# ODD2/DFD-CLIP

Hardware: AMD Instinct MI355X
Metric: 1-sec clips/sec (30x224x224 frames) ViT-B/16 (higher is better)
Workload: dtype bf16

## Files before the change

### dfd-clip_amd/capi.py

```python
import ctypes
import os
from ctypes import POINTER, Structure, c_char_p, c_float, c_int, c_int32, c_int64, c_size_t, c_uint32, c_void_p

import torch

PKG_DIR = os.path.dirname(os.path.abspath(__file__))
LIB_PATH = os.path.join(PKG_DIR, "libdfdclip_hip.so")

F32, BF16 = 0, 1
EPI_BIAS, EPI_BIAS_QUICKGELU, EPI_BIAS_RESIDUAL, EPI_PATCH_EMBED, EPI_QKV_EXPORT, EPI_RESIDUAL_POS, EPI_BIAS_GELU = range(7)
ABI_VERSION = 17

_DTYPE = {torch.float32: F32, torch.bfloat16: BF16}
FP8 = 2
FP8_MAX = 448.0
FP8_MIN_ROWS = 1024


class DfdError(RuntimeError):
    pass


GEMM_STREAM_OUT = 1
GEMM_SPARE_IF_FREE = 2


class GemmExtra(Structure):
    _fields_ = [("pos", c_void_p), ("cls", c_void_p), ("k_export", c_void_p), ("v_export", c_void_p),
                ("tokens", c_int32), ("frames_per_clip", c_int32), ("residual", c_void_p), ("qkv_first", c_int32),
                ("drop_rng", c_void_p), ("drop_site", c_uint32), ("drop_p", c_float), ("flags", c_uint32)]


class DropoutDesc(Structure):
    _fields_ = [("rng_state", c_void_p), ("site", c_uint32), ("p", c_float)]


class Dropout:
    __slots__ = ("rng", "site", "p")

# ... 196 lines not shown
    _profile["events"] = []
    _profile["base"] = None
    if epilogue is not None:
        _profile["base"] = torch.cuda.Event(enable_timing=True)
        _profile["base"].record()


def profile_gemm_collect():
    base = _profile["base"]
    spans = [(base.elapsed_time(a), base.elapsed_time(b), flops) for a, b, flops in _profile["events"]]
    profile_gemm(None)
    return spans


def gemm(a, w, c, bias=None, epilogue=EPI_BIAS, m=None, pos=None, cls=None, k_export=None, v_export=None, tokens=0,
         frames_per_clip=0, residual=None, qkv_first=0, drop=None, stream_out=False, spare_cus=0, tile_blocks=0, spare_if_free=False):
    _dev(a, w, c, bias, pos, cls, k_export, v_export, residual)
    assert a.dtype == w.dtype and a.stride(1) == 1 and w.stride(1) == 1 and c.stride(1) == 1
    M = a.shape[0] if m is None else m
    N, K = w.shape
    assert a.shape[1] == K
    assert residual is None or (residual.dtype == c.dtype and residual.stride(0) == c.stride(0))
    assert drop is None or epilogue == EPI_RESIDUAL_POS
    assert 0 <= epilogue <= EPI_BIAS_GELU, f"unknown epilogue {epilogue}"
    extra = GemmExtra(_ptr(pos).value, _ptr(cls).value, _ptr(k_export).value, _ptr(v_export).value, tokens, frames_per_clip,
                      _ptr(residual).value, qkv_first, drop.rng.data_ptr() if drop is not None and drop.p > 0 else None,
                      drop.site if drop is not None else 0, drop.p if drop is not None else 0.0, (GEMM_STREAM_OUT if stream_out else 0) | (GEMM_SPARE_IF_FREE if spare_if_free else 0) | ((int(spare_cus) & 0xff) << 8) | ((int(tile_blocks) & 0xf) << 16))
    timed = _profile["epilogue"] == epilogue
    if timed:
        e0, e1 = torch.cuda.Event(enable_timing=True), torch.cuda.Event(enable_timing=True)
        e0.record()
    _check(load_library().dfd_gemm(_ptr(a), a.stride(0), _ptr(w), w.stride(0), _DTYPE[a.dtype], _ptr(c), c.stride(0),
                                   _DTYPE[c.dtype], _ptr(bias), epilogue, ctypes.byref(extra), M, N, K, _stream()), "dfd_gemm")
    if timed:
        e1.record()
        _profile["events"].append((e0, e1, 2.0 * M * N * K))
    return c


def gemm_fp8(a, w, c, col_scale, bias=None, epilogue=EPI_BIAS, m=None, out_inv_scale=0.0, pos=None, k_export=None, v_export=None,
             tokens=0, frames_per_clip=0, qkv_first=0, stream_out=False, spare_cus=0, spare_if_free=False):
    _dev(a, w, c, col_scale, bias, pos, k_export, v_export)
# ... 363 lines not shown
```

### dfd-clip_amd/csrc/gemm.hip

```cpp
#include "gemm_args.hpp"
#include "gelu.hpp"

namespace {

constexpr int BM = 128, BN = 128;
constexpr int ROW_BYTES = 64;
constexpr int ROW_STRIDE = 80;
constexpr int TILE_BYTES = BM * ROW_STRIDE;
constexpr int EPI_SPLITK_SLAB = 100;

template <typename CT> __device__ __forceinline__ void store_c(void* C, int64_t off, float v) {
  static_cast<CT*>(C)[off] = from_f32<CT>(v);
}

template <typename CT, int EPI>
__device__ __forceinline__ void epilogue_elem(const GemmArgs& a, int64_t m, int n, float acc) {
  if (m >= a.M || n >= a.N) return;
  if constexpr (EPI == DFD_EPI_BIAS) {
    store_c<CT>(a.C, m * a.ldc + n, acc + (a.bias ? a.bias[n] : 0.f));
  } else if constexpr (EPI == DFD_EPI_BIAS_QUICKGELU) {
    store_c<CT>(a.C, m * a.ldc + n, quick_gelu(acc + (a.bias ? a.bias[n] : 0.f)));
  } else if constexpr (EPI == DFD_EPI_BIAS_GELU) {
    store_c<CT>(a.C, m * a.ldc + n, gelu_erf(acc + (a.bias ? a.bias[n] : 0.f)));
  } else if constexpr (EPI == DFD_EPI_BIAS_RESIDUAL) {
// ... 250 lines not shown
    DFD_REQUIRE(!extra->k_export == !extra->v_export, "dfd_gemm: QKV_EXPORT needs both k_export and v_export or neither");
    DFD_REQUIRE(!extra->pos || extra->frames_per_clip > 0, "dfd_gemm: QKV_EXPORT with pos needs frames_per_clip");
  }
  if (epilogue == DFD_EPI_RESIDUAL_POS) {
    DFD_REQUIRE(extra && extra->tokens > 1, "dfd_gemm: RESIDUAL_POS needs extra.tokens (patches per frame + 1)");
    DFD_REQUIRE(!extra->pos || extra->frames_per_clip > 0, "dfd_gemm: RESIDUAL_POS with pos needs frames_per_clip");
  }
  if (extra) {
    a.pos = extra->pos; a.cls = extra->cls; a.k_export = extra->k_export; a.v_export = extra->v_export;
    a.residual = epilogue == DFD_EPI_RESIDUAL_POS ? extra->residual : nullptr;
    a.tokens = extra->tokens; a.frames_per_clip = extra->frames_per_clip > 0 ? extra->frames_per_clip : 1;
    a.qkv_first = epilogue == DFD_EPI_QKV_EXPORT ? extra->qkv_first : 0;
    a.stream_out = (extra->flags & DFD_GEMM_STREAM_OUT) ? 1 : 0;
    a.spare_cus = (int)((extra->flags >> DFD_GEMM_SPARE_CUS_SHIFT) & 0xff);
    a.spare_if_free = (extra->flags & DFD_GEMM_SPARE_IF_FREE) ? 1 : 0;
    a.tile_rows = 32 * (int)((extra->flags >> DFD_GEMM_TILE_BLOCKS_SHIFT) & 0xf);
    DFD_REQUIRE(a.tile_rows == 0 || a.tile_rows == 224 || a.tile_rows == 256, "dfd_gemm: tile blocks must be 0, 7 or 8");
    if (epilogue == DFD_EPI_RESIDUAL_POS && extra->drop_rng && extra->drop_p > 0.f) {
      DFD_REQUIRE(extra->drop_p < 1.f, "dfd_gemm: drop_p=%f", (double)extra->drop_p);
      const dfd_dropout_t dd{extra->drop_rng, extra->drop_site, extra->drop_p};
      a.drop = dfd_make_drop(&dd);
    }
  }
  return DFD_OK;
}

static thread_local int g_last_path = 0;
static thread_local int g_gemm_variant = 0;
extern "C" int dfd_gemm_last_path(void) { return g_last_path; }
extern "C" int dfd_gemm_set_variant(int variant) {
// ... 11 lines not shown
  DFD_REQUIRE(c_dtype == DFD_F32 || c_dtype == DFD_BF16, "dfd_gemm: c_dtype=%d", c_dtype);
  DFD_REQUIRE(!(ab_dtype == DFD_F32 && c_dtype == DFD_BF16), "dfd_gemm: f32 operands with bf16 output unsupported");
  DFD_REQUIRE(K % 32 == 0, "dfd_gemm: K=%d must be a multiple of 32", K);
  const int esz = ab_dtype == DFD_F32 ? 4 : 2;
  DFD_REQUIRE(lda >= K && ldw >= K && (lda * esz) % 16 == 0 && (ldw * esz) % 16 == 0, "dfd_gemm: lda=%lld ldw=%lld must be >= K and 16-byte multiples", (long long)lda, (long long)ldw);
  DFD_REQUIRE(dfd_aligned16(A) && dfd_aligned16(W), "dfd_gemm: A and W must be 16-byte aligned");
  GemmArgs a{};
  a.A = A; a.W = W; a.C = C; a.bias = bias;
  a.lda = lda; a.ldw = ldw; a.ldc = ldc; a.M = M; a.N = N; a.K = K;
  { const int rc = fill_extra(a, epilogue, extra, c_dtype, ldc, M, N); if (rc != DFD_OK) return rc; }
  if (M == 0) return DFD_OK;
  hipStream_t st = static_cast<hipStream_t>(stream);
  if (ab_dtype == DFD_BF16) {
    const int epi_p = epilogue == DFD_EPI_QKV_EXPORT && a.k_export == nullptr ? DFD_EPI_BIAS : epilogue;
    a.no_dynamic = g_gemm_variant != 3;
    int rc = g_gemm_variant == 1 ? 1 : dfd_gemm256e_try(a, c_dtype, epi_p, st);
    if (rc == 0) g_last_path = 257;
    if (rc <= 0) return rc;
    rc = dfd_gemm256p_try(a, c_dtype, epi_p, st);
    if (rc == 0) g_last_path = 256;
    if (rc <= 0) return rc;
    rc = dfd_gemm256_try(a, c_dtype, epilogue, st);
    if (rc == 0) g_last_path = 256;
    if (rc <= 0) return rc;
  }
  g_last_path = 128;
  if (ab_dtype == DFD_F32) return launch_gemm128<float, float>(a, epilogue, st);
  if (c_dtype == DFD_BF16) return launch_gemm128<bf16_t, bf16_t>(a, epilogue, st);
  return launch_gemm128<bf16_t, float>(a, epilogue, st);
}

extern "C" int dfd_gemm_fp8(const void* A, int64_t lda, const void* W, int64_t ldw, void* C, int64_t ldc, int c_dtype,
                            const float* col_scale, const float* bias, float out_inv_scale, int epilogue,
                            const dfd_gemm_extra* extra, int64_t M, int N, int K, void* stream) {
// ... 59 lines not shown
```

### dfd-clip_amd/csrc/gemm256e.hip

```cpp
#include <mutex>
#include <unordered_map>

#include "gemm256p_common.hpp"
#include "gelu.hpp"

namespace {

constexpr int UNIT = 128 * ROWB;
constexpr int DEPTH = 6;
constexpr int NB = 2 * (DEPTH - 1);

template <int EPI, int RB, bool F8, bool CF8>
__global__ __launch_bounds__(512) void gemm256e_kernel(const GemmArgs a, int tiles_m, int tiles_n) {
  static_assert(!F8 || RB == 8, "fp8 form: 256-row tiles only");
  static_assert(!CF8 || (F8 && EPI != DFD_EPI_QKV_EXPORT), "fp8 output: fp8 operands, plain or QuickGELU epilogue");
  constexpr int ESZ = F8 ? 1 : 2;
  constexpr int CSZ = CF8 ? 1 : 2;
  constexpr int TMU = 32 * RB;
  constexpr int WROWS = 16 * RB;
  constexpr int HB = RB - 4;
  constexpr int NCV = F8 ? 2 : 1;
  constexpr int S1 = CF8 ? RB : 2 * RB;
  constexpr int S2 = 4 * RB;
  __shared__ __attribute__((aligned(1024))) unsigned char smem[RING + 8 * STAGE];
  const int tid = threadIdx.x;
  const int lane = tid & 63;
  const int wave = __builtin_amdgcn_readfirstlane(tid >> 6);
  const int wr = wave >> 2, wc = wave & 3;
  const int ntiles = tiles_m * tiles_n;

  const int G = gridDim.x, bid = blockIdx.x;
  const int xcd = bid & 7, q8 = G >> 3, r8 = G & 7;
  const int pos = (xcd < r8 ? xcd * (q8 + 1) : r8 * (q8 + 1) + (xcd - r8) * q8) + (bid >> 3);

  const __amdgpu_buffer_rsrc_t srdA = __builtin_amdgcn_make_buffer_rsrc(const_cast<void*>(a.A), 0, (int)(uint32_t)(a.M * a.lda * ESZ), 0x00020000);
  const __amdgpu_buffer_rsrc_t srdW = __builtin_amdgcn_make_buffer_rsrc(const_cast<void*>(a.W), 0, (int)(uint32_t)((int64_t)a.N * a.ldw * ESZ), 0x00020000);
  const __amdgpu_buffer_rsrc_t srdC = __builtin_amdgcn_make_buffer_rsrc(a.C, 0, (int)(uint32_t)(a.M * a.ldc * CSZ), 0x00020000);
  auto words = [](const float* p, int bytes) {
    const uint64_t u = reinterpret_cast<uint64_t>(p);
    return v4i{(int)(uint32_t)u, (int)((uint32_t)(u >> 32) & 0xffffu), bytes, 0x00020000};
  };
  const v4i srdB = words(a.bias ? a.bias : reinterpret_cast<const float*>(a.W), a.bias ? a.N * 4 : 0);
  [[maybe_unused]] const v4i srdS = words(F8 ? a.col_scale : reinterpret_cast<const float*>(a.W), F8 ? a.N * 4 : 0);
  const int cnt_x = q8 + (xcd < r8 ? 1 : 0), off_x = pos - (bid >> 3);
  const v4i srdT = words(reinterpret_cast<const float*>(a.sched ? a.sched : reinterpret_cast<const uint32_t*>(a.W)), a.sched ? 8 * 128 : 0);

  const uint32_t lda2 = (uint32_t)(a.lda * ESZ), ldw2 = (uint32_t)(a.ldw * ESZ);
  const uint32_t a_last = (uint32_t)(a.M - 1) * lda2;
  uint32_t vA[2][2], vW[2];
  auto set_a = [&](const Tile& t, int ha) {
    int l = lane;
    asm volatile("" : "+v"(l));
// ... 75 lines not shown
      for (int ks = 0; ks < 2; ++ks)
#pragma unroll
        for (int i = 0; i < (ha == 0 ? 4 : HB); ++i)
#pragma unroll
          for (int j = 0; j < 2; ++j)
            acc[4 * ha + i][2 * hb + j] = __builtin_amdgcn_mfma_f32_16x16x32_bf16(chunk(w[j], ks), chunk(Aa[i], ks), acc[4 * ha + i][2 * hb + j], 0, 0, 0);
    }
    __builtin_amdgcn_s_setprio(0);
    __builtin_amdgcn_sched_barrier(0);
    __builtin_amdgcn_s_barrier();
    __builtin_amdgcn_sched_barrier(0);
  };

  const int nk = a.K / (F8 ? 128 : TK);
  int idx = pos;
  Tile cur = decode_tile(idx, tiles_m, tiles_n, TMU);
  set_a(cur, 0);
  set_a(cur, 1);
  set_w(cur, 0);
  set_w(cur, 1);
#pragma unroll
  for (int v = 0; v <= DEPTH; ++v) issue(v & 3, v >> 2);
  wait_vm<NB>();
  __builtin_amdgcn_s_barrier();
  if (wr == 1) __builtin_amdgcn_s_barrier();
  __builtin_amdgcn_sched_barrier(0);
  int s_prev = 0;

  [[maybe_unused]] unsigned char* const ep = smem + RING + wave * STAGE;
  const int D = EPI == DFD_EPI_QKV_EXPORT ? a.N / (3 - a.qkv_first) : 0;
  [[maybe_unused]] __amdgpu_buffer_rsrc_t srdK = srdC, srdV = srdC, srdP = srdC;
// ... 1 lines not shown
    if (a.k_export != nullptr) {
      srdP = __builtin_amdgcn_make_buffer_rsrc(const_cast<float*>(a.pos ? a.pos : reinterpret_cast<const float*>(a.W)), 0,
                                               a.pos ? a.frames_per_clip * D * 4 : 0, 0x00020000);
      const int64_t erows = (a.M / a.tokens) * (a.tokens - 1);
      srdK = __builtin_amdgcn_make_buffer_rsrc(a.k_export, 0, (int)(uint32_t)(erows * D * 2), 0x00020000);
      srdV = __builtin_amdgcn_make_buffer_rsrc(a.v_export, 0, (int)(uint32_t)(erows * D * 2), 0x00020000);
    }
  }

  const int nk_ = a.K / (F8 ? 128 : TK);
  const bool dyn = !F8 && a.sched != nullptr && nk_ >= 6;
  const bool drawer = dyn && wave == 0;
  for (;;) {
    int nidx = idx + G;
    bool has_next = nidx < ntiles;
    Tile nxt = has_next ? decode_tile(nidx, tiles_m, tiles_n, TMU) : cur;
    uint32_t drawn = 1;
    if (drawer) {
      const uint32_t coff = (uint32_t)(xcd * 128);
      uint64_t saved_exec;
      asm volatile(
          "s_mov_b64 %1, exec\n\t"
          "s_mov_b64 exec, 1\n\t"
          "s_nop 4\n\t"
          "buffer_atomic_add %0, %2, %3, 0 offen sc0\n\t"
          "s_mov_b64 exec, %1"
          : "+v"(drawn), "=&s"(saved_exec)
          : "v"(coff), "s"(srdT)
          : "memory");
    }
#pragma unroll
// ... 99 lines not shown
        ktile(2, C0{}, C2{}, C1{});
        ktile(3, C1{}, C2{}, C0{});
      }
    } else {
      ktile(0, C0{}, C0{}, C4{});
      ktile(1, C1{}, C1{}, C4{});
      if (dyn) {
        uint32_t n;
        const uint32_t slot_addr = (uint32_t)(uintptr_t)(lds_ptr_t)(smem + RING + 1024);
        asm volatile("ds_read_b32 %0, %1\n\ts_waitcnt lgkmcnt(0)" : "=&v"(n) : "v"(slot_addr) : "memory");
        n = (uint32_t)__builtin_amdgcn_readfirstlane((int)n) - a.sched_base[xcd];
        const uint32_t r = n / (uint32_t)cnt_x;
        has_next = r < (uint32_t)(ntiles / G + 1);
        nidx = (int)((r + 1) * (uint32_t)G + (uint32_t)off_x + (n - r * (uint32_t)cnt_x));
        has_next = has_next && nidx < ntiles;
        nxt = has_next ? decode_tile(nidx, tiles_m, tiles_n, TMU) : cur;
      }
      for (int kt = 2; kt < nk - 4; kt += 2) {
        ktile(kt, C0{}, C2{}, C4{});
        ktile(kt + 1, C1{}, C2{}, C4{});
      }
      ktile(nk - 4, C0{}, C2{}, C3{});
      ktile(nk - 3, C1{}, C2{}, C2{});
      ktile(nk - 2, C0{}, C2{}, C1{});
      ktile(nk - 1, C1{}, C2{}, C0{});
    }

    int le = lane;
    asm volatile("" : "+v"(le));
    const int er = le & 15, eq = le >> 4;
    const int drow = le >> 3, dc = le & 7;
// ... 6 lines not shown
    int stores = 2 * RB;
    {
      f32x4 b4[4];
      [[maybe_unused]] f32x4 cs4[4];
#pragma unroll
      for (int j = 0; j < 4; ++j) {
        b4[j] = *reinterpret_cast<const f32x4*>(ep + (j * 16 + eq * 4) * 4);
        if constexpr (F8) cs4[j] = *reinterpret_cast<const f32x4*>(ep + 256 + (j * 16 + eq * 4) * 4);
      }
      asm volatile("s_waitcnt lgkmcnt(0)" ::: "memory");
#pragma unroll
      for (int i = 0; i < RB; ++i)
#pragma unroll
        for (int j = 0; j < 4; ++j) {
          if constexpr (F8) acc[i][j] = acc[i][j] * cs4[j] + b4[j];
          else acc[i][j] += b4[j];
        }
      if constexpr (EPI == DFD_EPI_QKV_EXPORT) {
        if (exporting) {
          stores = 4 * RB;
          const int ecol = nb - (which - a.qkv_first) * D + dc * 8;
          unsigned char* const parkf = ep + er * 256;
          const __amdgpu_buffer_rsrc_t srdE = which == 2 ? srdV : srdK;
#pragma unroll
          for (int i = 0; i < RB; ++i) {
            __builtin_amdgcn_sched_barrier(0);
            uint32_t eoff[2];
            f32x4 pe[2][2];
#pragma unroll
            for (int rr = 0; rr < 2; ++rr) {
              const int rloc = i * 16 + rr * 8;
// ... 97 lines not shown
            for (int e = 0; e < 4; ++e) {
              dv[e] = x0[e];
              dv[4 + e] = x1[e];
            }
            dfd_drop_eight(a.drop, (uint64_t)gq[b][rr] << 3, dv);
            const bf16x8 ob = __builtin_bit_cast(bf16x8, oq[b][rr]);
            bf16x8 o;
#pragma unroll
            for (int e = 0; e < 4; ++e) {
              o[e] = (bf16_t)((float)ob[e] + dv[e] + pq[b][rr][0][e]);
              o[4 + e] = (bf16_t)((float)ob[4 + e] + dv[4 + e] + pq[b][rr][1][e]);
            }
            store_out(__builtin_bit_cast(v4i, o), srdC, offq[b][rr], a.stream_out);
          }
        }
      } else if constexpr (CF8) {
        stores = RB;
        const int srow = le >> 2, sc = le & 3;
        unsigned char* const park8 = ep + er * 64 + eq * 4;
        const int psw = (er >> 1) & 3;
        const unsigned char* const dsrc8 = ep + srow * 64 + ((sc ^ ((srow >> 1) & 3)) << 4);
        const int64_t m8 = (int64_t)cur.m0 + wr * WROWS + srow;
        const int rows_left8 = (int)min((int64_t)0x7fffffff, a.M - m8);
        const uint32_t cbase8 = (uint32_t)(m8 * a.ldc + nb + sc * 16);
#pragma unroll
        for (int q = 0; q < 4; ++q) {
#pragma unroll
          for (int ii = 0; ii < 2; ++ii) {
            const int i = 2 * q + ii;
#pragma unroll
// ... 110 lines not shown
  if (n_cu == 0) {
    int dev = 0;
    hipDeviceProp_t prop;
    if (hipGetDevice(&dev) != hipSuccess || hipGetDeviceProperties(&prop, dev) != hipSuccess) {
      dfd_set_error("dfd_gemm(ping-pong): cannot query the device");
      return DFD_ERR_LAUNCH;
    }
    n_cu = prop.multiProcessorCount;
  }
  int cus = n_cu - a.spare_cus;
  cus = cus < n_cu / 2 ? n_cu / 2 : cus;
  if (a.spare_cus > 0 && a.spare_if_free) {
    auto cost = [&](int c) {
      auto r = [&](int rows) { return (double)((((a.M + rows - 1) / rows) * tiles_n + c - 1) / c); };
      const double r256 = r(256), r224 = r(224) * 0.97;
      return (F8 || EPI == DFD_EPI_RESIDUAL_POS) ? (EPI == DFD_EPI_RESIDUAL_POS ? r224 : r256) : (r224 < r256 ? r224 : r256);
    };
    if (cost(cus) > cost(n_cu)) cus = n_cu;
  }
  auto rounds = [&](int rows) {
    const int64_t tiles = ((a.M + rows - 1) / rows) * tiles_n;
    return (double)((tiles + cus - 1) / cus);
  };
  const bool use224 = !F8 && (EPI == DFD_EPI_RESIDUAL_POS || a.tile_rows == 224 || (a.tile_rows == 0 && rounds(224) * 0.97 < rounds(256)));
  const int rows = use224 ? 224 : 256;
  const int tiles_m = (int)((a.M + rows - 1) / rows);
  const int64_t ntiles = (int64_t)tiles_m * tiles_n;
  const int grid = (int)(ntiles < cus ? ntiles : cus);
  const int nk = a.K / (F8 ? 128 : TK);
  if (!F8 && nk >= 6 && a.no_dynamic == 0) sched_prepare(a, st, grid, ntiles);
  else a.sched = nullptr;
  if constexpr (F8) {
    hipLaunchKernelGGL((gemm256e_kernel<EPI, 8, true, CF8>), dim3(grid), dim3(512), 0, st, a, tiles_m, tiles_n);
  } else {
    if (use224) hipLaunchKernelGGL((gemm256e_kernel<EPI, 7, false, false>), dim3(grid), dim3(512), 0, st, a, tiles_m, tiles_n);
    else if constexpr (EPI != DFD_EPI_RESIDUAL_POS) hipLaunchKernelGGL((gemm256e_kernel<EPI, 8, false, false>), dim3(grid), dim3(512), 0, st, a, tiles_m, tiles_n);
  }
  hipError_t e = hipGetLastError();
  if (e != hipSuccess) {
    dfd_set_error("dfd_gemm(ping-pong): launch failed: %s", hipGetErrorString(e));
    return DFD_ERR_LAUNCH;
  }
  return DFD_OK;
}

int check256e(const GemmArgs& a, int esz, int csz, int kstep, bool short_k_ok = false) {
  const int nk = a.K / kstep;
  if (a.N % TN != 0 || a.K % kstep != 0 || (nk < 6 && !(short_k_ok && nk == 4)) || (nk & 1) || a.M < 1024) return 1;
  if ((a.ldw * esz) % 128 != 0) return 1;
  if ((a.lda * esz) % 16 != 0 || (a.ldw * esz) % 16 != 0 || (a.ldc * csz) % 16 != 0) return 1;
  if ((reinterpret_cast<uintptr_t>(a.A) & 15) != 0 || (reinterpret_cast<uintptr_t>(a.W) & 15) != 0 || (reinterpret_cast<uintptr_t>(a.C) & 15) != 0) return 1;
// ... 17 lines not shown
  if (c_dtype != DFD_BF16 || check256e(a, 2, 2, 64, epi == DFD_EPI_RESIDUAL_POS)) return 1;
  switch (epi) {
    case DFD_EPI_BIAS:
      return launch256e<DFD_EPI_BIAS, false, false>(a, st);
    case DFD_EPI_BIAS_QUICKGELU:
      return launch256e<DFD_EPI_BIAS_QUICKGELU, false, false>(a, st);
    case DFD_EPI_BIAS_GELU:
      return launch256e<DFD_EPI_BIAS_GELU, false, false>(a, st);
    case DFD_EPI_QKV_EXPORT: {
      if (check_export_e(a)) return 1;
      GemmArgs b = a;
      b.div_tokens = FastDiv::make((uint32_t)a.tokens);
      b.div_frames = FastDiv::make((uint32_t)a.frames_per_clip);
      return launch256e<DFD_EPI_QKV_EXPORT, false, false>(b, st);
    }
    case DFD_EPI_RESIDUAL_POS: {
      if (check256e(a, 2, 2, 64, true) || a.tokens < 2 || a.M * (int64_t)(a.N >> 3) >= ((int64_t)1 << 32)) return 1;
      if (a.pos && ((reinterpret_cast<uintptr_t>(a.pos) & 15) != 0 || a.frames_per_clip < 1)) return 1;
      if (a.residual && (reinterpret_cast<uintptr_t>(a.residual) & 15) != 0) return 1;
      GemmArgs b = a;
      b.div_tokens = FastDiv::make((uint32_t)(a.tokens - 1));
      b.div_frames = FastDiv::make((uint32_t)(a.frames_per_clip > 0 ? a.frames_per_clip : 1));
      return launch256e<DFD_EPI_RESIDUAL_POS, false, false>(b, st);
    }
    default:
      return 1;
  }
}

int dfd_gemm256e_f8_try(const GemmArgs& a, int c_dtype, int epi, hipStream_t st) {
  if (c_dtype != DFD_BF16 && c_dtype != DFD_FP8) return 1;
  if (!a.col_scale || (reinterpret_cast<uintptr_t>(a.col_scale) & 15) != 0) return 1;
  if (check256e(a, 1, c_dtype == DFD_FP8 ? 1 : 2, 128)) return 1;
  switch (epi) {
    case DFD_EPI_BIAS:
      return c_dtype == DFD_FP8 ? launch256e<DFD_EPI_BIAS, true, true>(a, st) : launch256e<DFD_EPI_BIAS, true, false>(a, st);
    case DFD_EPI_BIAS_QUICKGELU:
      return c_dtype == DFD_FP8 ? launch256e<DFD_EPI_BIAS_QUICKGELU, true, true>(a, st) : launch256e<DFD_EPI_BIAS_QUICKGELU, true, false>(a, st);
    case DFD_EPI_QKV_EXPORT: {
      if (c_dtype != DFD_BF16 || check_export_e(a)) return 1;
      GemmArgs b = a;
      b.div_tokens = FastDiv::make((uint32_t)a.tokens);
      b.div_frames = FastDiv::make((uint32_t)a.frames_per_clip);
      return launch256e<DFD_EPI_QKV_EXPORT, true, false>(b, st);
    }
    default:
      return 1;
  }
}
```

### dfd-clip_amd/csrc/gemm256p.hip

```cpp
#include "gemm256p_common.hpp"

namespace {

template <int EPI, int RB, bool F8, bool CF8>
__global__ __launch_bounds__(512) void gemm256p_kernel(const GemmArgs a, int tiles_m, int tiles_n) {
  static_assert(!F8 || RB == 8, "fp8 form: 256-row tiles only");
  static_assert(!CF8 || (F8 && EPI != DFD_EPI_QKV_EXPORT), "fp8 output: fp8 operands, plain or QuickGELU epilogue");
  constexpr int ESZ = F8 ? 1 : 2;
  constexpr int CSZ = CF8 ? 1 : 2;
  constexpr int TMU = 32 * RB;
  constexpr int WROWS = 16 * RB;
  constexpr int HB = RB - 4;
  __shared__ __attribute__((aligned(1024))) unsigned char smem[RING + 8 * STAGE];
  const int tid = threadIdx.x;
  const int lane = tid & 63;
  const int wave = __builtin_amdgcn_readfirstlane(tid >> 6);
  const int wr = wave >> 2, wc = wave & 3;
  const int ntiles = tiles_m * tiles_n;

  const int G = gridDim.x, bid = blockIdx.x;
  const int xcd = bid & 7, q8 = G >> 3, r8 = G & 7;
  const int pos = (xcd < r8 ? xcd * (q8 + 1) : r8 * (q8 + 1) + (xcd - r8) * q8) + (bid >> 3);

  const __amdgpu_buffer_rsrc_t srdA = __builtin_amdgcn_make_buffer_rsrc(const_cast<void*>(a.A), 0, (int)(uint32_t)(a.M * a.lda * ESZ), 0x00020000);
// ... 78 lines not shown
  };
  [[maybe_unused]] auto read_a8 = [&](v8i (&f)[2], int slot, int q) {
    const unsigned char* sb = smem + slot * SLOT + q * 32 * ROWB;
#pragma unroll
    for (int i = 0; i < 2; ++i) {
      const v4i x0 = *reinterpret_cast<const v4i*>(sb + offA[0] + i * 16 * ROWB), x1 = *reinterpret_cast<const v4i*>(sb + offA[1] + i * 16 * ROWB);
      f[i] = v8i{x0[0], x0[1], x0[2], x0[3], x1[0], x1[1], x1[2], x1[3]};
    }
  };
  [[maybe_unused]] auto mfma8 = [&](const v8i& w, const v8i& f, f32x4 c) {
    return __builtin_amdgcn_mfma_scale_f32_16x16x128_f8f6f4(w, f, c, 0, 0, 0, 0x7f7f7f7f, 0, 0x7f7f7f7f);
  };

  const int nk = a.K / (F8 ? 128 : TK);
  int idx = pos;
  Tile cur = decode_tile(idx, tiles_m, tiles_n, TMU);
  set_a(cur);
  set_w(cur);
  int par = 0;
  issue_a(0, 0);
  issue_w(0, 0);
  issue_a(1, 1);
  issue_w(1, 1);
  wait_vm<8>();
  __builtin_amdgcn_s_barrier();
  int s_prev = 0;

  [[maybe_unused]] bf16x8 wA[4], wB[4], lo[4], hi[4];
  [[maybe_unused]] v8i W8[4], aE[2], aO[2];
  [[maybe_unused]] unsigned char* const ep = smem + RING + wave * STAGE;
  const int D = EPI == DFD_EPI_QKV_EXPORT ? a.N / (3 - a.qkv_first) : 0;
  [[maybe_unused]] __amdgpu_buffer_rsrc_t srdK = srdC, srdV = srdC, srdP = srdC;
  if constexpr (EPI == DFD_EPI_QKV_EXPORT) {
    if (a.k_export != nullptr) {
      srdP = __builtin_amdgcn_make_buffer_rsrc(const_cast<float*>(a.pos ? a.pos : reinterpret_cast<const float*>(a.W)), 0,
                                               a.pos ? a.frames_per_clip * D * 4 : 0, 0x00020000);
      const int64_t erows = (a.M / a.tokens) * (a.tokens - 1);
      srdK = __builtin_amdgcn_make_buffer_rsrc(a.k_export, 0, (int)(uint32_t)(erows * D * 2), 0x00020000);
      srdV = __builtin_amdgcn_make_buffer_rsrc(a.v_export, 0, (int)(uint32_t)(erows * D * 2), 0x00020000);
    }
  }

  for (;;) {
    const int nidx = idx + G;
    const bool has_next = nidx < ntiles;
    const Tile nxt = has_next ? decode_tile(nidx, tiles_m, tiles_n, TMU) : cur;
#pragma unroll
    for (int i = 0; i < RB; ++i)
#pragma unroll
      for (int j = 0; j < 4; ++j) acc[i][j] = f32x4{0.f, 0.f, 0.f, 0.f};
    if constexpr (F8) {
#pragma unroll
      for (int j = 0; j < 4; ++j) read_w8(W8, par, j);
      read_a8(aE, par, 0);
    } else {
      read_w(wA, par, 0);
      read_a(lo, par, 0, 0);
    }
    f32x4 b4[4];
    [[maybe_unused]] f32x4 cs4[4];

// ... 383 lines not shown
```

### dfd-clip_amd/csrc/gemm256p_common.hpp

```cpp
#pragma once
#include <type_traits>

#include "gemm_args.hpp"

typedef int v4i_t __attribute__((ext_vector_type(4)));
typedef v4i_t v4i;
typedef int v8i __attribute__((ext_vector_type(8)));

namespace {

__device__ __forceinline__ void store_out(v4i_t d, __amdgpu_buffer_rsrc_t srd, uint32_t off, int stream_out) {
  if (stream_out) {
    __builtin_amdgcn_raw_buffer_store_b128(d, srd, off, 0, 2);
  } else {
    __builtin_amdgcn_raw_buffer_store_b128(d, srd, off, 0, 0);
  }
}

constexpr int TM = 256, TN = 256, TK = 64;
constexpr int ROWB = TK * 2;
constexpr int A_BYTES = TM * ROWB;
constexpr int SLOT = (TM + TN) * ROWB;
constexpr int RING = 2 * SLOT;
constexpr int STAGE = 4096;
typedef __attribute__((address_space(3))) void* lds_ptr_t;

struct Tile {
  int m0, n0;
};

__device__ __forceinline__ Tile decode_tile(int idx, int tiles_m, int tiles_n, int tile_rows) {
  const int ngroups = (tiles_n + 5) / 6;
  const int gcols = (tiles_n + ngroups - 1) / ngroups;
  int grp = idx / (tiles_m * gcols);
  grp = grp < ngroups - 1 ? grp : ngroups - 1;
  const int rem = idx - grp * tiles_m * gcols;
  const int cols_here = min(gcols, tiles_n - grp * gcols);
  const int tm = rem / cols_here, tn = grp * gcols + (rem - tm * cols_here);
  return Tile{tm * tile_rows, tn * TN};
}

template <int N> __device__ __forceinline__ void wait_vm() { asm volatile("s_waitcnt vmcnt(%0)" ::"n"(N) : "memory"); }

}
```

### dfd-clip_amd/csrc/gemm_args.hpp

```cpp
#pragma once
#include "dropout.hpp"

struct GemmArgs {
  const void* A;
  const void* W;
  void* C;
  const float* bias;
  const float* pos;
  const float* cls;
  void* k_export;
  void* v_export;
  const void* residual;
  int64_t lda, ldw, ldc, M;
  int N, K, tokens, frames_per_clip;
  int qkv_first;
  int stream_out;
  int spare_cus;
  int spare_if_free;
  int tile_rows;
  DfdDrop drop;
  FastDiv div_tokens, div_frames;
  const float* col_scale;
  float out_inv_scale;
  uint32_t* sched;
  uint32_t sched_base[8];
  int no_dynamic;
};

int dfd_gemm256_try(const GemmArgs& a, int c_dtype, int epi, hipStream_t st);
int dfd_gemm256p_try(const GemmArgs& a, int c_dtype, int epi, hipStream_t st);
int dfd_gemm256p_f8_try(const GemmArgs& a, int c_dtype, int epi, hipStream_t st);
int dfd_gemm256e_try(const GemmArgs& a, int c_dtype, int epi, hipStream_t st);
int dfd_gemm256e_f8_try(const GemmArgs& a, int c_dtype, int epi, hipStream_t st);
```

### dfd-clip_amd/encoder.py

```python
import contextlib

import torch
from torch import nn

from . import capi


class RuntimeStateMixin:
    _RUNTIME_STATE = {}

    def __deepcopy__(self, memo):
        import copy
        new = self.__class__.__new__(self.__class__)
        memo[id(self)] = new
        for k, v in self.__dict__.items():
            if k in self._RUNTIME_STATE:
                new.__dict__[k] = copy.deepcopy(self._RUNTIME_STATE[k])
            else:
                new.__dict__[k] = copy.deepcopy(v, memo)
        return new


class _Holder(nn.Module):

# ... 238 lines not shown
            assert x.dim() == 4 and x.shape[1] == 3, "uint8 frames must be [N, 3, H, W]"
            return x.contiguous()
        assert tuple(x.shape[1:]) == (3, self.input_resolution, self.input_resolution), \
            f"frames must be [N, 3, {self.input_resolution}, {self.input_resolution}]"
        return x.to(torch.float32).contiguous()

    def _embed(self, frames, ws, p):
        n = frames.shape[0]
        P, D = self.tokens - 1, self.width
        if frames.dtype == torch.uint8:
            capi.preprocess_u8(frames, ws["patches"][:n * P], self.input_resolution, self.patch_size, self.pixel_mean,
                               self.pixel_std, antialias=self.antialias)
        else:
            capi.patchify(frames, ws["patches"], self.input_resolution, self.patch_size)
        capi.gemm(ws["patches"], p["w_patch"], ws["x"], None, capi.EPI_PATCH_EMBED, m=n * P, pos=p["pos"], cls=p["cls"],
                  tokens=self.tokens)
        ws["pending"] = 0
        ws["ln_pre"] = p["ln_pre"]

    def _ln(self, ws, gb, M, store=True, q=None, discard_x=False):
        x = ws["x"]
        h, inv = (ws["h8"], q) if q is not None else (ws["h"], 0.0)
        pend = ws.get("pending", 0)
        pre = ws.pop("ln_pre", None)
        if pre is not None:
            assert pend == 0
            if self.width <= 2048:
                capi.layernorm2(x[:M], pre[0], pre[1], gb[0], gb[1], h[:M], eps=self.ln_eps, out_inv_scale=inv)
            else:
                capi.layernorm(x[:M], pre[0], pre[1], x[:M], eps=self.ln_eps)
                capi.layernorm(x[:M], gb[0], gb[1], h[:M], eps=self.ln_eps, out_inv_scale=inv)
# ... 163 lines not shown
```

### include/dfdclip.h

```cpp
#ifndef DFDCLIP_H
#define DFDCLIP_H

#include <stddef.h>
#include <stdint.h>

#ifdef __cplusplus
extern "C" {
#endif

#define DFD_ABI_VERSION 17

enum { DFD_F32 = 0, DFD_BF16 = 1, DFD_FP8 = 2  };

enum {
  DFD_OK = 0,
  DFD_ERR_INVALID_ARG = -1,
  DFD_ERR_LAUNCH = -2,
  DFD_ERR_NO_DEVICE = -3
};

enum {
  DFD_EPI_BIAS = 0,
  DFD_EPI_BIAS_QUICKGELU,
  DFD_EPI_BIAS_RESIDUAL,
// ... 15 lines not shown
  void* k_export;
  void* v_export;
  int32_t tokens;
  int32_t frames_per_clip;
  const void* residual;
  int32_t qkv_first;
  const uint64_t* drop_rng;
  uint32_t drop_site;
  float drop_p;
  uint32_t flags;
} dfd_gemm_extra;

enum {
  DFD_GEMM_STREAM_OUT = 1,
  DFD_GEMM_SPARE_IF_FREE = 2,
  DFD_GEMM_TILE_BLOCKS_SHIFT = 16,
  DFD_GEMM_SPARE_CUS_SHIFT = 8
};

const char* dfd_last_error(void);
int dfd_abi_version(void);
int dfd_device_check(void);

int dfd_layernorm(const float* x, int64_t ldx, const float* gamma, const float* beta, void* y, int64_t ldy,
                  int y_dtype, int64_t rows, int cols, float eps, float y_inv_scale, void* stream);

int dfd_layernorm2(float* x, int64_t ldx, const float* gamma_a, const float* beta_a, const float* gamma_b, const float* beta_b,
                   void* y, int64_t ldy, int y_dtype, int64_t rows, int cols, float eps, float y_inv_scale, void* stream);

int dfd_add_layernorm(float* x, int64_t ldx, const void* delta, const void* delta2, int64_t ldd, int delta_dtype,
// ... 129 lines not shown
```

Baseline: 870.8.

## Route patch-embed GEMM through ping-pong 256e kernel with fused pos/cls epilogue

Adds a PATCH_EMBED epilogue to the gemm256e persistent kernel. It writes fp32 outputs plus positional embeddings and inserts the cls+pos row for each frame, so the patch-embedding GEMM can use the faster ping-pong path instead of falling back to older kernels. The encoder enables it through a new flag. Tile decoding is also changed to put the partial last M-panel at the end of the schedule in both the 256e and 256p kernels, which affects every GEMM. The change adds a debug tile-order helper and extra per-row division and loads in the epilogue.

```diff
diff --git a/dfd-clip_amd/capi.py b/dfd-clip_amd/capi.py
--- a/dfd-clip_amd/capi.py
+++ b/dfd-clip_amd/capi.py
@@ -23,6 +23,7 @@
 
 GEMM_STREAM_OUT = 1
 GEMM_SPARE_IF_FREE = 2
+GEMM_PATCH_PINGPONG = 4
 
 
 class GemmExtra(Structure):
@@ -249,7 +250,8 @@
 
 
 def gemm(a, w, c, bias=None, epilogue=EPI_BIAS, m=None, pos=None, cls=None, k_export=None, v_export=None, tokens=0,
-         frames_per_clip=0, residual=None, qkv_first=0, drop=None, stream_out=False, spare_cus=0, tile_blocks=0, spare_if_free=False):
+         frames_per_clip=0, residual=None, qkv_first=0, drop=None, stream_out=False, spare_cus=0, tile_blocks=0, spare_if_free=False,
+         patch_pingpong=False):
     _dev(a, w, c, bias, pos, cls, k_export, v_export, residual)
     assert a.dtype == w.dtype and a.stride(1) == 1 and w.stride(1) == 1 and c.stride(1) == 1
     M = a.shape[0] if m is None else m
@@ -260,7 +262,7 @@
     assert 0 <= epilogue <= EPI_BIAS_GELU, f"unknown epilogue {epilogue}"
     extra = GemmExtra(_ptr(pos).value, _ptr(cls).value, _ptr(k_export).value, _ptr(v_export).value, tokens, frames_per_clip,
                       _ptr(residual).value, qkv_first, drop.rng.data_ptr() if drop is not None and drop.p > 0 else None,
-                      drop.site if drop is not None else 0, drop.p if drop is not None else 0.0, (GEMM_STREAM_OUT if stream_out else 0) | (GEMM_SPARE_IF_FREE if spare_if_free else 0) | ((int(spare_cus) & 0xff) << 8) | ((int(tile_blocks) & 0xf) << 16))
+                      drop.site if drop is not None else 0, drop.p if drop is not None else 0.0, (GEMM_STREAM_OUT if stream_out else 0) | (GEMM_SPARE_IF_FREE if spare_if_free else 0) | (GEMM_PATCH_PINGPONG if patch_pingpong else 0) | ((int(spare_cus) & 0xff) << 8) | ((int(tile_blocks) & 0xf) << 16))
     timed = _profile["epilogue"] == epilogue
     if timed:
         e0, e1 = torch.cuda.Event(enable_timing=True), torch.cuda.Event(enable_timing=True)
diff --git a/dfd-clip_amd/csrc/gemm.hip b/dfd-clip_amd/csrc/gemm.hip
--- a/dfd-clip_amd/csrc/gemm.hip
+++ b/dfd-clip_amd/csrc/gemm.hip
@@ -288,6 +288,7 @@
     a.stream_out = (extra->flags & DFD_GEMM_STREAM_OUT) ? 1 : 0;
     a.spare_cus = (int)((extra->flags >> DFD_GEMM_SPARE_CUS_SHIFT) & 0xff);
     a.spare_if_free = (extra->flags & DFD_GEMM_SPARE_IF_FREE) ? 1 : 0;
+    a.patch_pingpong = (extra->flags & DFD_GEMM_PATCH_PINGPONG) ? 1 : 0;
     a.tile_rows = 32 * (int)((extra->flags >> DFD_GEMM_TILE_BLOCKS_SHIFT) & 0xf);
     DFD_REQUIRE(a.tile_rows == 0 || a.tile_rows == 224 || a.tile_rows == 256, "dfd_gemm: tile blocks must be 0, 7 or 8");
     if (epilogue == DFD_EPI_RESIDUAL_POS && extra->drop_rng && extra->drop_p > 0.f) {
@@ -329,10 +330,11 @@
   if (ab_dtype == DFD_BF16) {
     const int epi_p = epilogue == DFD_EPI_QKV_EXPORT && a.k_export == nullptr ? DFD_EPI_BIAS : epilogue;
     a.no_dynamic = g_gemm_variant != 3;
-    int rc = g_gemm_variant == 1 ? 1 : dfd_gemm256e_try(a, c_dtype, epi_p, st);
+    int rc = g_gemm_variant == 1 || g_gemm_variant == 2 ? 1 : dfd_gemm256e_try(a, c_dtype, epi_p, st);
+    if (rc == 1 && epilogue == DFD_EPI_PATCH_EMBED && a.patch_pingpong && g_gemm_variant != 1 && g_gemm_variant != 2) rc = dfd_gemm256e_patch_try(a, c_dtype, st);
     if (rc == 0) g_last_path = 257;
     if (rc <= 0) return rc;
-    rc = dfd_gemm256p_try(a, c_dtype, epi_p, st);
+    rc = g_gemm_variant == 2 ? 1 : dfd_gemm256p_try(a, c_dtype, epi_p, st);
     if (rc == 0) g_last_path = 256;
     if (rc <= 0) return rc;
     rc = dfd_gemm256_try(a, c_dtype, epilogue, st);
diff --git a/dfd-clip_amd/csrc/gemm256e.hip b/dfd-clip_amd/csrc/gemm256e.hip
--- a/dfd-clip_amd/csrc/gemm256e.hip
+++ b/dfd-clip_amd/csrc/gemm256e.hip
@@ -15,12 +15,12 @@
   static_assert(!F8 || RB == 8, "fp8 form: 256-row tiles only");
   static_assert(!CF8 || (F8 && EPI != DFD_EPI_QKV_EXPORT), "fp8 output: fp8 operands, plain or QuickGELU epilogue");
   constexpr int ESZ = F8 ? 1 : 2;
-  constexpr int CSZ = CF8 ? 1 : 2;
+  constexpr int CSZ = CF8 ? 1 : (EPI == DFD_EPI_PATCH_EMBED ? 4 : 2);
   constexpr int TMU = 32 * RB;
   constexpr int WROWS = 16 * RB;
   constexpr int HB = RB - 4;
   constexpr int NCV = F8 ? 2 : 1;
-  constexpr int S1 = CF8 ? RB : 2 * RB;
+  constexpr int S1 = CF8 ? RB : (EPI == DFD_EPI_PATCH_EMBED ? 4 * RB : 2 * RB);
   constexpr int S2 = 4 * RB;
   __shared__ __attribute__((aligned(1024))) unsigned char smem[RING + 8 * STAGE];
   const int tid = threadIdx.x;
@@ -28,6 +28,7 @@
   const int wave = __builtin_amdgcn_readfirstlane(tid >> 6);
   const int wr = wave >> 2, wc = wave & 3;
   const int ntiles = tiles_m * tiles_n;
+  const int full_m = full_panels(a.M, tiles_m, 32 * RB);
 
   const int G = gridDim.x, bid = blockIdx.x;
   const int xcd = bid & 7, q8 = G >> 3, r8 = G & 7;
@@ -35,7 +36,8 @@
 
   const __amdgpu_buffer_rsrc_t srdA = __builtin_amdgcn_make_buffer_rsrc(const_cast<void*>(a.A), 0, (int)(uint32_t)(a.M * a.lda * ESZ), 0x00020000);
   const __amdgpu_buffer_rsrc_t srdW = __builtin_amdgcn_make_buffer_rsrc(const_cast<void*>(a.W), 0, (int)(uint32_t)((int64_t)a.N * a.ldw * ESZ), 0x00020000);
-  const __amdgpu_buffer_rsrc_t srdC = __builtin_amdgcn_make_buffer_rsrc(a.C, 0, (int)(uint32_t)(a.M * a.ldc * CSZ), 0x00020000);
+  const int64_t c_rows = EPI == DFD_EPI_PATCH_EMBED ? a.M / (a.tokens - 1) * a.tokens : a.M;
+  const __amdgpu_buffer_rsrc_t srdC = __builtin_amdgcn_make_buffer_rsrc(a.C, 0, (int)(uint32_t)(c_rows * a.ldc * CSZ), 0x00020000);
   auto words = [](const float* p, int bytes) {
     const uint64_t u = reinterpret_cast<uint64_t>(p);
     return v4i{(int)(uint32_t)u, (int)((uint32_t)(u >> 32) & 0xffffu), bytes, 0x00020000};
@@ -141,7 +143,7 @@
 
   const int nk = a.K / (F8 ? 128 : TK);
   int idx = pos;
-  Tile cur = decode_tile(idx, tiles_m, tiles_n, TMU);
+  Tile cur = decode_tile(idx, full_m, tiles_n, TMU);
   set_a(cur, 0);
   set_a(cur, 1);
   set_w(cur, 0);
@@ -173,7 +175,7 @@
   for (;;) {
     int nidx = idx + G;
     bool has_next = nidx < ntiles;
-    Tile nxt = has_next ? decode_tile(nidx, tiles_m, tiles_n, TMU) : cur;
+    Tile nxt = has_next ? decode_tile(nidx, full_m, tiles_n, TMU) : cur;
     uint32_t drawn = 1;
     if (drawer) {
       const uint32_t coff = (uint32_t)(xcd * 128);
@@ -303,7 +305,7 @@
         has_next = r < (uint32_t)(ntiles / G + 1);
         nidx = (int)((r + 1) * (uint32_t)G + (uint32_t)off_x + (n - r * (uint32_t)cnt_x));
         has_next = has_next && nidx < ntiles;
-        nxt = has_next ? decode_tile(nidx, tiles_m, tiles_n, TMU) : cur;
+        nxt = has_next ? decode_tile(nidx, full_m, tiles_n, TMU) : cur;
       }
       for (int kt = 2; kt < nk - 4; kt += 2) {
         ktile(kt, C0{}, C2{}, C4{});
@@ -340,7 +342,7 @@
 #pragma unroll
         for (int j = 0; j < 4; ++j) {
           if constexpr (F8) acc[i][j] = acc[i][j] * cs4[j] + b4[j];
-          else acc[i][j] += b4[j];
+          else if constexpr (EPI != DFD_EPI_PATCH_EMBED) acc[i][j] += b4[j];
         }
       if constexpr (EPI == DFD_EPI_QKV_EXPORT) {
         if (exporting) {
@@ -468,6 +470,56 @@
             store_out(__builtin_bit_cast(v4i, o), srdC, offq[b][rr], a.stream_out);
           }
         }
+      } else if constexpr (EPI == DFD_EPI_PATCH_EMBED) {
+        stores = 4 * RB;
+        const uint32_t P = (uint32_t)(a.tokens - 1);
+        const uint32_t ncol = (uint32_t)(nb + dc * 8);
+        const __amdgpu_buffer_rsrc_t srdQ = __builtin_amdgcn_make_buffer_rsrc(const_cast<float*>(a.pos), 0, a.tokens * a.N * 4, 0x00020000);
+        const __amdgpu_buffer_rsrc_t srdL = __builtin_amdgcn_make_buffer_rsrc(const_cast<float*>(a.cls), 0, a.N * 4, 0x00020000);
+        unsigned char* const parkf = ep + er * 256;
+#pragma unroll
+        for (int g8 = 0; g8 < 2 * RB; ++g8) {
+          const int rloc = g8 * 8;
+          const uint32_t m = (uint32_t)min(mrow0 + rloc, a.M - 1);
+          const uint32_t frame = a.div_tokens.div(m);
+          const bool first = rloc < rows_left && m == frame * P;
+          if (__builtin_amdgcn_ballot_w64(first) != 0) {
+            const f32x4 c0 = __builtin_bit_cast(f32x4, __builtin_amdgcn_raw_buffer_load_b128(srdL, ncol * 4, 0, 0)) +
+                             __builtin_bit_cast(f32x4, __builtin_amdgcn_raw_buffer_load_b128(srdQ, ncol * 4, 0, 0));
+            const f32x4 c1 = __builtin_bit_cast(f32x4, __builtin_amdgcn_raw_buffer_load_b128(srdL, ncol * 4, 16, 0)) +
+                             __builtin_bit_cast(f32x4, __builtin_amdgcn_raw_buffer_load_b128(srdQ, ncol * 4, 16, 0));
+            const uint32_t off = first ? (frame * (uint32_t)a.tokens * (uint32_t)a.ldc + ncol) * 4 : 0xffffffffu;
+            __builtin_amdgcn_raw_buffer_store_b128(__builtin_bit_cast(v4i, c0), srdC, off, 0, 0);
+            __builtin_amdgcn_raw_buffer_store_b128(__builtin_bit_cast(v4i, c1), srdC, off + (first ? 16u : 0u), 0, 0);
+          }
+        }
+#pragma unroll
+        for (int i = 0; i < RB; ++i) {
+          __builtin_amdgcn_sched_barrier(0);
+          uint32_t coff[2];
+          f32x4 pe[2][2];
+#pragma unroll
+          for (int rr = 0; rr < 2; ++rr) {
+            const int rloc = i * 16 + rr * 8;
+            const uint32_t m = (uint32_t)min(mrow0 + rloc, a.M - 1);
+            const uint32_t frame = a.div_tokens.div(m);
+            const uint32_t tok = m - frame * P + 1;
+            coff[rr] = rloc < rows_left ? ((frame * (uint32_t)a.tokens + tok) * (uint32_t)a.ldc + ncol) * 4 : 0xffffffffu;
+            const uint32_t poff = (tok * (uint32_t)a.N + ncol) * 4;
+            pe[rr][0] = __builtin_bit_cast(f32x4, __builtin_amdgcn_raw_buffer_load_b128(srdQ, poff, 0, 0));
+            pe[rr][1] = __builtin_bit_cast(f32x4, __builtin_amdgcn_raw_buffer_load_b128(srdQ, poff, 16, 0));
+          }
+#pragma unroll
+          for (int j = 0; j < 4; ++j) *reinterpret_cast<f32x4*>(parkf + (((j * 4 + eq) ^ er) << 4)) = acc[i][j];
+#pragma unroll
+          for (int rr = 0; rr < 2; ++rr) {
+            const int row = rr * 8 + drow;
+            const f32x4 x0 = *reinterpret_cast<const f32x4*>(ep + row * 256 + (((2 * dc) ^ row) << 4)) + pe[rr][0];
+            const f32x4 x1 = *reinterpret_cast<const f32x4*>(ep + row * 256 + (((2 * dc + 1) ^ row) << 4)) + pe[rr][1];
+            store_out(__builtin_bit_cast(v4i, x0), srdC, coff[rr], a.stream_out);
+            store_out(__builtin_bit_cast(v4i, x1), srdC, coff[rr] + (coff[rr] == 0xffffffffu ? 0u : 16u), a.stream_out);
+          }
+        }
       } else if constexpr (CF8) {
         stores = RB;
         const int srow = le >> 2, sc = le & 3;
@@ -608,7 +660,8 @@
     auto cost = [&](int c) {
       auto r = [&](int rows) { return (double)((((a.M + rows - 1) / rows) * tiles_n + c - 1) / c); };
       const double r256 = r(256), r224 = r(224) * 0.97;
-      return (F8 || EPI == DFD_EPI_RESIDUAL_POS) ? (EPI == DFD_EPI_RESIDUAL_POS ? r224 : r256) : (r224 < r256 ? r224 : r256);
+      constexpr bool only224 = EPI == DFD_EPI_RESIDUAL_POS || EPI == DFD_EPI_PATCH_EMBED;
+      return (F8 || only224) ? (only224 ? r224 : r256) : (r224 < r256 ? r224 : r256);
     };
     if (cost(cus) > cost(n_cu)) cus = n_cu;
   }
@@ -616,7 +669,7 @@
     const int64_t tiles = ((a.M + rows - 1) / rows) * tiles_n;
     return (double)((tiles + cus - 1) / cus);
   };
-  const bool use224 = !F8 && (EPI == DFD_EPI_RESIDUAL_POS || a.tile_rows == 224 || (a.tile_rows == 0 && rounds(224) * 0.97 < rounds(256)));
+  const bool use224 = !F8 && (EPI == DFD_EPI_RESIDUAL_POS || EPI == DFD_EPI_PATCH_EMBED || a.tile_rows == 224 || (a.tile_rows == 0 && rounds(224) * 0.97 < rounds(256)));
   const int rows = use224 ? 224 : 256;
   const int tiles_m = (int)((a.M + rows - 1) / rows);
   const int64_t ntiles = (int64_t)tiles_m * tiles_n;
@@ -628,7 +681,7 @@
     hipLaunchKernelGGL((gemm256e_kernel<EPI, 8, true, CF8>), dim3(grid), dim3(512), 0, st, a, tiles_m, tiles_n);
   } else {
     if (use224) hipLaunchKernelGGL((gemm256e_kernel<EPI, 7, false, false>), dim3(grid), dim3(512), 0, st, a, tiles_m, tiles_n);
-    else if constexpr (EPI != DFD_EPI_RESIDUAL_POS) hipLaunchKernelGGL((gemm256e_kernel<EPI, 8, false, false>), dim3(grid), dim3(512), 0, st, a, tiles_m, tiles_n);
+    else if constexpr (EPI != DFD_EPI_RESIDUAL_POS && EPI != DFD_EPI_PATCH_EMBED) hipLaunchKernelGGL((gemm256e_kernel<EPI, 8, false, false>), dim3(grid), dim3(512), 0, st, a, tiles_m, tiles_n);
   }
   hipError_t e = hipGetLastError();
   if (e != hipSuccess) {
@@ -676,6 +729,8 @@
       b.div_frames = FastDiv::make((uint32_t)a.frames_per_clip);
       return launch256e<DFD_EPI_QKV_EXPORT, false, false>(b, st);
     }
+    case DFD_EPI_PATCH_EMBED:
+      return 1;
     case DFD_EPI_RESIDUAL_POS: {
       if (check256e(a, 2, 2, 64, true) || a.tokens < 2 || a.M * (int64_t)(a.N >> 3) >= ((int64_t)1 << 32)) return 1;
       if (a.pos && ((reinterpret_cast<uintptr_t>(a.pos) & 15) != 0 || a.frames_per_clip < 1)) return 1;
@@ -688,6 +743,18 @@
     default:
       return 1;
   }
+}
+
+int dfd_gemm256e_patch_try(const GemmArgs& a, int c_dtype, hipStream_t st) {
+  if (c_dtype != DFD_F32 || a.tokens < 2 || !a.pos || !a.cls || a.M % (a.tokens - 1) != 0) return 1;
+  GemmArgs b = a;
+  b.M = a.M / (a.tokens - 1) * a.tokens;
+  if (check256e(b, 2, 4, 64) || a.M < 1024) return 1;
+  if ((reinterpret_cast<uintptr_t>(a.pos) & 15) != 0 || (reinterpret_cast<uintptr_t>(a.cls) & 15) != 0) return 1;
+  if ((int64_t)a.tokens * a.N * 4 > (int64_t)0x7ffffff0) return 1;
+  b.M = a.M;
+  b.div_tokens = FastDiv::make((uint32_t)(a.tokens - 1));
+  return launch256e<DFD_EPI_PATCH_EMBED, false, false>(b, st);
 }
 
 int dfd_gemm256e_f8_try(const GemmArgs& a, int c_dtype, int epi, hipStream_t st) {
@@ -710,3 +777,16 @@
       return 1;
   }
 }
+
+extern "C" int64_t dfd_debug_gemm_tile_order(int64_t M, int N, int tile_rows, int32_t* panel, int32_t* column, int64_t capacity) {
+  if (M < 1 || N < TN || N % TN != 0 || (tile_rows != 224 && tile_rows != 256) || !panel || !column) return -1;
+  const int64_t tiles_m = (M + tile_rows - 1) / tile_rows, tiles_n = N / TN;
+  if (tiles_m * tiles_n > 0x3fffffff) return -1;
+  const int full_m = full_panels(M, (int)tiles_m, tile_rows);
+  for (int64_t idx = 0; idx < tiles_m * tiles_n && idx < capacity; ++idx) {
+    const Tile t = decode_tile((int)idx, full_m, (int)tiles_n, tile_rows);
+    panel[idx] = t.m0 / tile_rows;
+    column[idx] = t.n0 / TN;
+  }
+  return tiles_m * tiles_n;
+}
diff --git a/dfd-clip_amd/csrc/gemm256p.hip b/dfd-clip_amd/csrc/gemm256p.hip
--- a/dfd-clip_amd/csrc/gemm256p.hip
+++ b/dfd-clip_amd/csrc/gemm256p.hip
@@ -116,7 +116,8 @@
 
   const int nk = a.K / (F8 ? 128 : TK);
   int idx = pos;
-  Tile cur = decode_tile(idx, tiles_m, tiles_n, TMU);
+  const int full_m = full_panels(a.M, tiles_m, TMU);
+  Tile cur = decode_tile(idx, full_m, tiles_n, TMU);
   set_a(cur);
   set_w(cur);
   int par = 0;
@@ -146,7 +147,7 @@
   for (;;) {
     const int nidx = idx + G;
     const bool has_next = nidx < ntiles;
-    const Tile nxt = has_next ? decode_tile(nidx, tiles_m, tiles_n, TMU) : cur;
+    const Tile nxt = has_next ? decode_tile(nidx, full_m, tiles_n, TMU) : cur;
 #pragma unroll
     for (int i = 0; i < RB; ++i)
 #pragma unroll
diff --git a/dfd-clip_amd/csrc/gemm256p_common.hpp b/dfd-clip_amd/csrc/gemm256p_common.hpp
--- a/dfd-clip_amd/csrc/gemm256p_common.hpp
+++ b/dfd-clip_amd/csrc/gemm256p_common.hpp
@@ -29,13 +29,19 @@
   int m0, n0;
 };
 
-__device__ __forceinline__ Tile decode_tile(int idx, int tiles_m, int tiles_n, int tile_rows) {
+__host__ __device__ __forceinline__ int full_panels(int64_t M, int tiles_m, int tile_rows) {
+  return (int64_t)tiles_m * tile_rows > M ? tiles_m - 1 : tiles_m;
+}
+__host__ __device__ __forceinline__ Tile decode_tile(int idx, int full_m, int tiles_n, int tile_rows) {
+  const int nfull = full_m * tiles_n;
+  if (idx >= nfull) return Tile{full_m * tile_rows, (idx - nfull) * TN};
   const int ngroups = (tiles_n + 5) / 6;
   const int gcols = (tiles_n + ngroups - 1) / ngroups;
-  int grp = idx / (tiles_m * gcols);
+  int grp = idx / (full_m * gcols);
   grp = grp < ngroups - 1 ? grp : ngroups - 1;
-  const int rem = idx - grp * tiles_m * gcols;
-  const int cols_here = min(gcols, tiles_n - grp * gcols);
+  const int rem = idx - grp * full_m * gcols;
+  const int gleft = tiles_n - grp * gcols;
+  const int cols_here = gcols < gleft ? gcols : gleft;
   const int tm = rem / cols_here, tn = grp * gcols + (rem - tm * cols_here);
   return Tile{tm * tile_rows, tn * TN};
 }
diff --git a/dfd-clip_amd/csrc/gemm_args.hpp b/dfd-clip_amd/csrc/gemm_args.hpp
--- a/dfd-clip_amd/csrc/gemm_args.hpp
+++ b/dfd-clip_amd/csrc/gemm_args.hpp
@@ -25,10 +25,12 @@
   uint32_t* sched;
   uint32_t sched_base[8];
   int no_dynamic;
+  int patch_pingpong;
 };
 
 int dfd_gemm256_try(const GemmArgs& a, int c_dtype, int epi, hipStream_t st);
 int dfd_gemm256p_try(const GemmArgs& a, int c_dtype, int epi, hipStream_t st);
 int dfd_gemm256p_f8_try(const GemmArgs& a, int c_dtype, int epi, hipStream_t st);
 int dfd_gemm256e_try(const GemmArgs& a, int c_dtype, int epi, hipStream_t st);
+int dfd_gemm256e_patch_try(const GemmArgs& a, int c_dtype, hipStream_t st);
 int dfd_gemm256e_f8_try(const GemmArgs& a, int c_dtype, int epi, hipStream_t st);
diff --git a/dfd-clip_amd/encoder.py b/dfd-clip_amd/encoder.py
--- a/dfd-clip_amd/encoder.py
+++ b/dfd-clip_amd/encoder.py
@@ -276,7 +276,7 @@
         else:
             capi.patchify(frames, ws["patches"], self.input_resolution, self.patch_size)
         capi.gemm(ws["patches"], p["w_patch"], ws["x"], None, capi.EPI_PATCH_EMBED, m=n * P, pos=p["pos"], cls=p["cls"],
-                  tokens=self.tokens)
+                  tokens=self.tokens, patch_pingpong=True)
         ws["pending"] = 0
         ws["ln_pre"] = p["ln_pre"]
 
diff --git a/include/dfdclip.h b/include/dfdclip.h
--- a/include/dfdclip.h
+++ b/include/dfdclip.h
@@ -53,6 +53,7 @@
 enum {
   DFD_GEMM_STREAM_OUT = 1,
   DFD_GEMM_SPARE_IF_FREE = 2,
+  DFD_GEMM_PATCH_PINGPONG = 4,
   DFD_GEMM_TILE_BLOCKS_SHIFT = 16,
   DFD_GEMM_SPARE_CUS_SHIFT = 8
 };
```

New measurement: 867.3. No clear change (-0.4%).
